# djeedai/bevy_hanabi

Measured on AMD Instinct MI355X. Metric: particle-updates/sec, higher is better.
Workload: dtype f32

## Files before the change

### bevy_hanabi_amd/csrc/hnb_kernels.hip.h

```cpp
#pragma once
#ifndef __HIPCC_RTC__
#include <hip/hip_runtime.h>
#endif
#include "hnb_dev.h"

namespace hnb {

template <class T>
__device__ __forceinline__ T* global_ptr(uint64_t addr) {
    typedef __attribute__((address_space(1))) T global_t;
    return (T*)(global_t*)addr;
}

struct u2_t { uint32_t x, y; };
struct u3_t { uint32_t x, y, z; };
typedef uint32_t u4v __attribute__((ext_vector_type(4)));
#if defined(HNB_NONTEMPORAL) || defined(HNB_NONTEMPORAL_LOADS)
#define HNB_NT_LOAD(p) __builtin_nontemporal_load(p)
#else
#define HNB_NT_LOAD(p) (*(p))
#endif
#if defined(HNB_NONTEMPORAL) || defined(HNB_NONTEMPORAL_STORES)
#define HNB_NT_STORE(v, p) __builtin_nontemporal_store(v, p)
#else
// ... 936 lines not shown
        }
        uint32_t incl = local;
#pragma unroll
        for (uint32_t off = 1; off < 64; off <<= 1) { const uint32_t y = __shfl_up(incl, off, 64); if (lane >= off) incl += y; }
        if (lane == 63) s_scan[wave] = incl;
        __syncthreads();
        uint32_t pos = excl + incl - local;
        for (uint32_t w = 0; w < wave; ++w) pos += s_scan[w];
#pragma unroll
        for (uint32_t r = 0; r < kPer; ++r) {
            if (n_ev[r] >= kEmitHeavy) {
                if ((tid * kPer + r) % n_split == split) {
                    const uint32_t h = atomicAdd(&s_heavy_n, 1u);
                    s_heavy[h][0] = slot[r]; s_heavy[h][1] = pos; s_heavy[h][2] = n_ev[r];
                }
            } else if (split == 0u) {
                const uint32_t end = pos + n_ev[r] < capacity ? pos + n_ev[r] : capacity;
                for (uint32_t e = pos; e < end; ++e) ev->data[e] = slot[r];
            }
            pos += n_ev[r];
        }
        __syncthreads();
        const uint32_t n_heavy = s_heavy_n;
        for (uint32_t h = 0; h < n_heavy; ++h) {
            const uint32_t sl = s_heavy[h][0], first = s_heavy[h][1];
            const uint32_t end = first + s_heavy[h][2] < capacity ? first + s_heavy[h][2] : capacity;
            for (uint32_t e = first + tid; e < end; e += kBlock) ev->data[e] = sl;
        }
        __syncthreads();
    }
}
#endif

#ifndef HNB_STREAM_WAVES
#define HNB_STREAM_WAVES 6
#endif
#ifndef HNB_STREAM_WAVES_FULL
#define HNB_STREAM_WAVES_FULL 5
#endif

template <bool B> struct BoolTag { static constexpr bool value = B; };
struct SlotArgs {
    uint32_t capacity, n_uregs, chunks_per_inst, n_inst;
    soff_t alive_flag_off;
    uint32_t update_len;
    soff_t plane_off[4];
    uint32_t flags;
    soff_t died_bits_off;
    uint32_t write_died;
    uint32_t cull_lifetime;
    soff_t lmin_off;
    uint32_t dt_operand;
    uint32_t age_cohort;
    soff_t horizon_off;
    uint32_t horizon;
    uint32_t frame_phase;
    const Ins* update_code;
    uint32_t* safe_words;
    unsigned long long* safe_host;
    uint32_t safe_parity, publish_tag, safe_stride;
    uint32_t skip_lists;
    const DevMeta* meta_in;
    DevMeta* meta_out;
    uint32_t* fault;
    uint32_t transpose;
    uint32_t stream_hint;
    uint32_t store_hint;
    uint32_t quarters;
    uint32_t age_current;
    uint32_t fuse_steps;
};




__device__ __forceinline__ void store_died_bits(uint32_t* __restrict__ bits, uint32_t step_first, uint32_t nib, uint32_t lane) {
    int v = (int)(nib << (4u * (lane & 7u)));
    v |= __builtin_amdgcn_update_dpp(0, v, 0xB1, 0xf, 0xf, true);
    v |= __builtin_amdgcn_update_dpp(0, v, 0x4E, 0xf, 0xf, true);
    v |= __builtin_amdgcn_update_dpp(0, v, 0x141, 0xf, 0xf, true);
    if ((lane & 7u) == 0u) bits[(step_first >> 5) + (lane >> 3)] = (uint32_t)v;
}

struct StreamLds {
    uint32_t died[kBlock / 64];
    float lmin[kBlock / 64];
    uint32_t alive[kBlock / 64];
    float rem[kBlock / 64];
    uint32_t amin[kBlock / 64], amax[kBlock / 64];
    u4v xp[2][kBlock / 64][kStepRows * 3u / 4u];
};
__device__ __forceinline__ StreamLds& stream_lds() {
    __shared__ StreamLds s;
    return s;
}

template <class PROG, int PROBE, bool COHORT, bool FUSED = false>
__device__ __forceinline__ void update_stream_chunk(const SlotArgs& args, const uint64_t* __restrict__ inst_base, const DevFrameInst* __restrict__ fi,
                                                    const uint32_t* __restrict__ ublocks, const CompactBufs& cb,
                                                    const uint32_t wg, const uint32_t wg_total) {
    StreamLds& lds = stream_lds();
    uint32_t (&s_died)[kBlock / 64] = lds.died;
    float (&s_lmin)[kBlock / 64] = lds.lmin;
    uint32_t (&s_alive)[kBlock / 64] = lds.alive;
    float (&s_rem)[kBlock / 64] = lds.rem;
    uint32_t (&s_amin)[kBlock / 64] = lds.amin;
    uint32_t (&s_amax)[kBlock / 64] = lds.amax;
    u4v (&s_xp)[2][kBlock / 64][kStepRows * 3u / 4u] = lds.xp;
    const uint32_t tid = threadIdx.x, lane = tid & 63u, wave = tid >> 6;
    const bool split = !FUSED && !COHORT && args.quarters == 4u;
    const uint32_t S = FUSED ? args.fuse_steps : 1u;
    const uint32_t chunk = split ? chunk_of_workgroup(cb.xcd_remap, wg >> 2, wg_total >> 2) : chunk_of_workgroup(cb.xcd_remap, wg, wg_total);
    const uint32_t quarter = split ? (wg & 3u) : 0u;
    const uint32_t k = chunk / args.chunks_per_inst, j = chunk - k * args.chunks_per_inst;
    const uint32_t wave0 = j * kChunk + (split ? (quarter * (kBlock / 64u) + wave) * kStepRows : wave * kWaveRows);
    const uint32_t n_steps = split ? 1u : kWaveRows / kStepRows;
    const uint32_t n_words = split ? wg_total >> 2 : wg_total;
    const uint32_t frozen = fi[k].skip;
    const uint64_t slab = inst_base[k];
    const bool store_nt = args.store_hint != 0u;
#ifndef HNB_PUBLISH_FIRST_WG
#define HNB_PUBLISH_FIRST_WG 1
#endif
    if (args.safe_words && (HNB_PUBLISH_FIRST_WG ? wg == 0u : chunk == 0u)) {
        uint32_t* prev = args.safe_words + (size_t)(args.safe_parity ^ 1u) * args.safe_stride;
        uint32_t m = 0x7f800000u;
        for (uint32_t i = tid; i < n_words; i += kBlock) { const uint32_t v = prev[i]; prev[i] = 0x7f800000u; m = v < m ? v : m; }
        m = wave_min_u32(m);
        if (lane == 0) s_alive[wave] = m;
        __syncthreads();
        if (tid == 0u) {
            for (uint32_t w = 1; w < kBlock / 64; ++w) m = s_alive[w] < m ? s_alive[w] : m;
            *reinterpret_cast<volatile unsigned long long*>(args.safe_host) = ((unsigned long long)m << 32) | (unsigned long long)args.publish_tag;
        }
        __syncthreads();
    }
    if (args.skip_lists && j == 0u && quarter == 0u && tid == 0u) {
        DevMeta o = args.meta_in[k];
        if constexpr (FUSED) {
            DevMeta before = o;
            if (!frozen) {
                o.max_update = o.alive_count; o.dead_count = 0u; o.spawned = 0u; o.instance_count = o.alive_count;
                before = o;
                o.ref_write_index ^= S & 1u;
                before.ref_write_index ^= (S - 1u) & 1u;
            }
            DevMeta* row_in = const_cast<DevMeta*>(args.meta_in);
            ((S & 1u) ? args.meta_out : row_in)[k] = o;
            ((S & 1u) ? row_in : args.meta_out)[k] = before;
            cb.deaths[(size_t)(cb.parity ^ 1u) * cb.table_cap + k] = 0u;
        } else {
        if (!frozen) {
            o.ref_write_index ^= 1u;
            o.max_update = o.alive_count; o.dead_count = 0u; o.spawned = 0u; o.instance_count = o.alive_count;
        }
        args.meta_out[k] = o;
        cb.deaths[(size_t)(cb.parity ^ 1u) * cb.table_cap + k] = 0u;
        }
    }
    if (frozen) return;
    char* base = global_ptr<char>(slab);
    VmUniforms U;
    U.u = ublocks + (size_t)k * args.n_uregs * S;
    auto uniforms_of = [&](const uint32_t s) { VmUniforms Us = U; Us.u = U.u + (size_t)s * args.n_uregs; return Us; };
    U.xf = fi[k].xf;
    float rem_min = __builtin_inff();
    char* p_pos = base + args.plane_off[0];
    char* p_vel = base + args.plane_off[1];
    char* p_age = base + args.plane_off[2];
    char* p_life = base + args.plane_off[3];
    uint32_t* flags4 = reinterpret_cast<uint32_t*>(base + args.alive_flag_off);
    const uint32_t fl = args.flags;
    uint32_t died_total = 0;
    uint32_t* cfull = reinterpret_cast<uint32_t*>(base + args.lmin_off) + args.chunks_per_inst;
    const bool chunk_full = cfull[j] == 1u;
    uint32_t* astate = cfull + args.chunks_per_inst;
    uint32_t* aval = astate + args.chunks_per_inst;
    const uint32_t ast_raw = COHORT ? astate[j] : 0u;
    bool check_due = ((args.frame_phase + j) & 15u) == 0u;
    if constexpr (FUSED) {
        for (uint32_t s = 1; s < S; ++s) check_due = check_due || ((args.frame_phase + s + j) & 15u) == 0u;
    }
    const bool mixed = COHORT && ast_raw == 4u && !check_due;
    const uint32_t ast = ast_raw == 4u ? 0u : ast_raw;
    const float A = COHORT ? u2f(aval[j]) : 0.0f;
    uint32_t amin = 0xffffffffu, amax = 0u;
    uint32_t lane_alive = 0;
    const bool cull = args.cull_lifetime != 0u;
    float* lmin = reinterpret_cast<float*>(base + args.lmin_off);
    const float Lm = cull ? lmin[j] : 0.0f;
    const float dt_tick = cull ? uf(U, args.dt_operand) : 0.0f;
    auto age_after = [&](float a) {
        if constexpr (FUSED) {
            for (uint32_t s = 0; s < S; ++s) a = a + uf(uniforms_of(s), args.dt_operand);
            return a;
        } else return a + dt_tick;
    };
    if (args.horizon && j == 0u && quarter == 0u && tid == 0u) {
        double* clk = horizon_view(base, args.horizon_off, args.chunks_per_inst).clock;
        if constexpr (FUSED) {
            double c = *clk;
            for (uint32_t s = 0; s < S; ++s) { const float t = cull ? uf(uniforms_of(s), args.dt_operand) : 0.0f; c = c + (double)(t > 0.0f ? t : 0.0f) * (1.0 + 0x1p-16); }
            *clk = c;
        } else
        *clk = *clk + (double)(dt_tick > 0.0f ? dt_tick : 0.0f) * (1.0 + 0x1p-16);
    }
    float wave_min = __builtin_inff();
    bool loaded_all = true;
    bool flat = false;
    if constexpr (PROG::kFlat && COHORT && PROBE == 0) {
        flat = chunk_full && ast == 1u && cull && Lm > 0.0f && (age_after(A) < Lm) && (fl & 3u) == 3u && !(fl & 128u);
    }
    if (flat) {
        if constexpr (PROG::kFlat && COHORT && PROBE == 0) {
            const float A2 = age_after(A);
            u4v* pw = reinterpret_cast<u4v*>(p_pos + (size_t)j * (kChunk * 12u)) + wave * (kWaveRows * 3u / 4u);
            u4v* vw = reinterpret_cast<u4v*>(p_vel + (size_t)j * (kChunk * 12u)) + wave * (kWaveRows * 3u / 4u);
            const uint32_t rot = lane % 3u;
            if (args.age_current && (fl & 64u)) {
                u4v* aw = reinterpret_cast<u4v*>(p_age + (size_t)j * (kChunk * 4u)) + wave * (kWaveRows / 4u);
                const uint32_t a2 = f2u(A2);
#pragma unroll
                for (uint32_t step = 0; step < kWaveRows / kStepRows; ++step) aw[step * 64u + lane] = u4v{a2, a2, a2, a2};
            }
#pragma unroll 2
            for (uint32_t step = 0; step < kWaveRows / kStepRows; ++step) {
                float P[3][4], V[3][4];
#pragma unroll
                for (uint32_t w = 0; w < 3; ++w) {
                    const u4v a = pw[(step * 3u + w) * 64u + lane], b = vw[(step * 3u + w) * 64u + lane];
                    P[w][0] = u2f(a.x); P[w][1] = u2f(a.y); P[w][2] = u2f(a.z); P[w][3] = u2f(a.w);
                    V[w][0] = u2f(b.x); V[w][1] = u2f(b.y); V[w][2] = u2f(b.z); V[w][3] = u2f(b.w);
                }
                if constexpr (FUSED) {
                    for (uint32_t s = 0; s < S; ++s) PROG::run_flat(args.update_code, P, V, rot, uniforms_of(s));
                } else
                PROG::run_flat(args.update_code, P, V, rot, U);
#pragma unroll
                for (uint32_t w = 0; w < 3; ++w) {
                    if (fl & 16u) pw[(step * 3u + w) * 64u + lane] = u4v{f2u(P[w][0]), f2u(P[w][1]), f2u(P[w][2]), f2u(P[w][3])};
                    if (fl & 32u) vw[(step * 3u + w) * 64u + lane] = u4v{f2u(V[w][0]), f2u(V[w][1]), f2u(V[w][2]), f2u(V[w][3])};
                }
            }
            if (args.write_died && lane < kWaveRows / 32u)
                reinterpret_cast<uint32_t*>(base + args.died_bits_off)[((j * kChunk + wave * kWaveRows) >> 5) + lane] = 0u;
            amin = amax = f2u(A2);
            loaded_all = false;
            if (args.safe_words) rem_min = (f2u(A2) >> 31) ? 0.0f : (Lm - A2) - 1.0e-5f * Lm;
        }
    }
    auto step_body = [&](auto coh_tag, const uint32_t step, const uint32_t f4, const u4v* pre_age = nullptr) {
        constexpr bool COH = decltype(coh_tag)::value;
        const uint32_t s0 = wave0 + step * kStepRows + lane * 4u;
        bool was[4], fresh[4];
#pragma unroll
        for (int p = 0; p < 4; ++p) {
            const uint32_t byte = (f4 >> (8 * p)) & 0xffu;
            fresh[p] = COH && byte == 3u;
            was[p] = byte == 1u || fresh[p];
            lane_alive += was[p] ? 1u : 0u;
        }
        const bool any = was[0] || was[1] || was[2] || was[3];
        if (!__any(any)) {
            if (args.write_died) store_died_bits(reinterpret_cast<uint32_t*>(base + args.died_bits_off), s0 - lane * 4u, 0u, lane);
            return;
        }
        const bool full = was[0] && was[1] && was[2] && was[3];
        uint32_t slot[4];
#pragma unroll
        for (int p = 0; p < 4; ++p) slot[p] = s0 + p;
        bool lanes_on[4] = {any, any, any, any};
        Pinned<4> X;
#pragma unroll
        for (int p = 0; p < 4; ++p) { X.pos[p] = V3{0, 0, 0}; X.vel[p] = V3{0, 0, 0}; X.age[p] = 0.0f; X.lifetime[p] = 0.0f; X.alive[p] = true; }
        bool need_life = true;
        float age_was[4] = {0.0f, 0.0f, 0.0f, 0.0f};
        const uint32_t step_first = s0 - lane * 4u;
        const bool xp = args.transpose != 0u && PROBE == 0 && step_first + kStepRows <= args.capacity && __popcll(__ballot(any)) >= 32;
        if (xp) {
            if (fl & 1u) xpose_load3(X.pos, p_pos, step_first, s_xp[0][wave], lane);
            if (fl & 2u) xpose_load3(X.vel, p_vel, step_first, s_xp[1][wave], lane);
        }
        if (any) {
            if (!xp) {
                if (fl & 1u) pin_load3<4>(X.pos, p_pos, slot, lanes_on, true);
                if (fl & 2u) pin_load3<4>(X.vel, p_vel, slot, lanes_on, true);
            }
            if (fl & 4u) {
                if (!COH || ast != 1u) {
                    if (pre_age) { X.age[0] = u2f(pre_age->x); X.age[1] = u2f(pre_age->y); X.age[2] = u2f(pre_age->z); X.age[3] = u2f(pre_age->w); }
                    else pin_load1<4>(X.age, p_age, slot, lanes_on, true);
                    for (int p = 0; p < 4; ++p) age_was[p] = X.age[p];
                }
                if (COH && ast != 0u) {
#pragma unroll
                    for (int p = 0; p < 4; ++p) X.age[p] = fresh[p] ? X.age[p] : A;
                }
            }
        }
        if (cull && Lm > 0.0f && (COH || !mixed)) {
            bool may_die = false;
#pragma unroll
            for (int p = 0; p < 4; ++p) may_die = may_die || (was[p] && !(age_after(X.age[p]) < Lm));
            need_life = __any(may_die);
        }
        if (any && (fl & 8u)) {
            if (need_life) {
                if (args.stream_hint) {
                    const u4v ql = __builtin_nontemporal_load(reinterpret_cast<const u4v*>(p_life) + (slot[0] >> 2));
                    X.lifetime[0] = u2f(ql.x); X.lifetime[1] = u2f(ql.y); X.lifetime[2] = u2f(ql.z); X.lifetime[3] = u2f(ql.w);
                } else pin_load1<4>(X.lifetime, p_life, slot, lanes_on, true);
            }
            else {
#pragma unroll
                for (int p = 0; p < 4; ++p) X.lifetime[p] = Lm;
            }
        }
        if (!need_life) loaded_all = false;
        if constexpr (FUSED) {
            bool gone[4] = {false, false, false, false};
            for (uint32_t s = 0; s < S; ++s) {
                PROG::template run<4>(args.update_code, args.update_len, X, uniforms_of(s));
#pragma unroll
                for (int p = 0; p < 4; ++p) gone[p] = gone[p] || !X.alive[p];
            }
#pragma unroll
            for (int p = 0; p < 4; ++p) X.alive[p] = !gone[p];
        } else
        if constexpr (!(PROBE & 8)) PROG::template run<4>(args.update_code, args.update_len, X, U);
        if constexpr (!(PROBE & 4)) {
            const bool xp_pos = xp && (fl & 17u) == 17u, xp_vel = xp && (fl & 34u) == 34u;
            if (xp_pos) xpose_store3(X.pos, p_pos, step_first, s_xp[0][wave], lane, was, full, store_nt);
            if (xp_vel) xpose_store3(X.vel, p_vel, step_first, s_xp[1][wave], lane, was, full, store_nt);
            if (any) {
                if ((fl & 16u) && !xp_pos) pin_store3<4>(X.pos, p_pos, slot, was, full);
                if ((fl & 32u) && !xp_vel) pin_store3<4>(X.vel, p_vel, slot, was, full);
                if (fl & 64u) {
                    const bool plane_loaded = !COH || ast != 1u;
                    if (plane_loaded || args.age_current) {
                        if (plane_loaded && (fl & 4u) && !full) {
                            float q[4];
#pragma unroll
                            for (int p = 0; p < 4; ++p) q[p] = was[p] ? X.age[p] : age_was[p];
                            pin_store1<4>(q, p_age, slot, was, true, store_nt);
                        } else pin_store1<4>(X.age, p_age, slot, was, full, store_nt);
                    }
                }
                if (fl & 128u) pin_store1<4>(X.lifetime, p_life, slot, was, full);
            }
        } else {
            float acc = 0.0f;
#pragma unroll
            for (int p = 0; p < 4; ++p) acc += X.pos[p].x + X.pos[p].y + X.pos[p].z + X.vel[p].x + X.vel[p].y + X.vel[p].z + X.age[p] + X.lifetime[p];
            if (acc == 123.456f) X.alive[0] = false;
        }
        if (cull && need_life) {
#pragma unroll
            for (int p = 0; p < 4; ++p)
                if (was[p] && X.alive[p]) wave_min = fminf(wave_min, X.lifetime[p]);
        }
        if (args.safe_words) {
#pragma unroll
            for (int p = 0; p < 4; ++p)
                if (was[p] && X.alive[p]) rem_min = fminf(rem_min, (f2u(X.age[p]) >> 31) ? 0.0f : (X.lifetime[p] - X.age[p]) - 1.0e-5f * X.lifetime[p]);
        }
        if constexpr (COH) {
#pragma unroll
            for (int p = 0; p < 4; ++p) {
                const bool stays = was[p] && X.alive[p];
                const uint32_t b = f2u(X.age[p]);
                amin = (stays && b < amin) ? b : amin;
                amax = (stays && b > amax) ? b : amax;
            }
            if constexpr (!(PROBE & 4)) {
                const bool dies = (was[0] && !X.alive[0]) || (was[1] && !X.alive[1]) || (was[2] && !X.alive[2]) || (was[3] && !X.alive[3]);
                if (ast == 1u && (fl & 64u) && !args.age_current && __any(dies)) {
#pragma unroll
                    for (int p = 0; p < 4; ++p)
                        if (was[p] && !X.alive[p]) reinterpret_cast<float*>(p_age)[slot[p]] = X.age[p];
                }
            }
        }
        uint32_t nf = f4, nib = 0u;
        uint32_t died_here = 0;
#pragma unroll
        for (int p = 0; p < 4; ++p) {
            const bool died = was[p] && !X.alive[p];
            if (died) { nf &= ~(0xffu << (8 * p)); nib |= 1u << p; }
            else if (COH && fresh[p]) nf = (nf & ~(0xffu << (8 * p))) | (1u << (8 * p));
            died_here += (uint32_t)__popcll(__ballot(died));
        }
        if (nf != f4) flags4[s0 >> 2] = nf;
        if (args.write_died) store_died_bits(reinterpret_cast<uint32_t*>(base + args.died_bits_off), step_first, nib, lane);
        died_total += died_here;
    };
    if (!flat) {
        auto f4_of = [&](const uint32_t step) {
            const uint32_t s0 = wave0 + step * kStepRows + lane * 4u;
            return chunk_full ? 0x01010101u : (s0 < args.capacity ? ld_hint(flags4 + (s0 >> 2), args.stream_hint != 0u) : 0u);
        };
        if constexpr (COHORT || PROG::kFlat) {
            uint32_t f4s[kWaveRows / kStepRows];
#pragma unroll
            for (uint32_t step = 0; step < kWaveRows / kStepRows; ++step) f4s[step] = step < n_steps ? f4_of(step) : 0u;
            if constexpr (PROG::kAgeOnly && !COHORT) {
                if ((fl & 4u) && !(fl & 3u)) {
                    u4v ages[kWaveRows / kStepRows];
#pragma unroll
                    for (uint32_t step = 0; step < kWaveRows / kStepRows; ++step) {
                        const uint32_t s0 = wave0 + step * kStepRows + lane * 4u;
                        ages[step] = (step < n_steps && s0 < args.capacity) ? reinterpret_cast<const u4v*>(p_age)[s0 >> 2] : u4v{0u, 0u, 0u, 0u};
                    }
// ... 524 lines not shown
```

### bevy_hanabi_amd/csrc/hnb_vm.h

```cpp
#pragma once
#include "hnb_math.h"
#ifdef __HIPCC_RTC__
#include "hanabi_amd.h"
#else
#include "../../include/hanabi_amd.h"
#endif

namespace hnb {

struct __attribute__((aligned(8))) Ins { uint32_t x, y; };

#ifdef HNB_VM_BOUNDS_CHECK
extern "C" void hnb_vm_oob(uint32_t index, uint32_t size);
template <uint32_t N>
struct checked_file_t {
    uint32_t v[N];
    uint32_t& operator[](uint32_t i) { if (i >= N) hnb_vm_oob(i, N); return v[i < N ? i : 0]; }
    const uint32_t& operator[](uint32_t i) const { if (i >= N) hnb_vm_oob(i, N); return v[i < N ? i : 0]; }
};
typedef checked_file_t<HNB_VM_MAX_REGS> vreg_file_t;
typedef checked_file_t<HNB_VM_MAX_REGS_WIDE> vreg_file_wide_t;
typedef checked_file_t<HNB_VM_MAX_UREGS> UFile;
#else
typedef uint32_t vreg_file_t __attribute__((vector_size(HNB_VM_MAX_REGS * 4)));
// ... 636 lines not shown
template <int P, bool FULL>
HNB_HD void fast_run(const Ins* __restrict__ code, uint32_t n_ins, Pinned<P>& X, const VmUniforms& U) {
    for (uint32_t pc = 0; pc < n_ins; ++pc) {
        const Ins ins = code[pc];
        const uint32_t op = ins.x & 0xffu, d = (ins.x >> 8) & 0xffu, aux = ins.y >> 16;
        const uint32_t a = HNB_OPERAND_DECODE((ins.x >> 16) & 0xffu, ins.y >> 13), b = HNB_OPERAND_DECODE(ins.x >> 24, ins.y >> 14);
        const uint32_t c = HNB_OPERAND_DECODE(ins.y & 0xffu, ins.y >> 15);
        switch (op) {
            case HNB_OP_M_AGE_TICK: {
                const float dt = uf(U, a);
#pragma unroll
                for (int p = 0; p < P; ++p) mac_age_tick(X.age[p], X.lifetime[p], dt, (aux & 1u) != 0u, X.alive[p]);
            } break;
            case HNB_OP_M_EULER: {
                const float dt = uf(U, a);
#pragma unroll
                for (int p = 0; p < P; ++p) mac_euler(X.pos[p], X.vel[p], dt);
            } break;
            case HNB_OP_M_VEL_SCALE: {
                const float s = uf(U, a);
#pragma unroll
                for (int p = 0; p < P; ++p) mac_vel_scale(X.vel[p], s);
            } break;
            case HNB_OP_M_VEL_ADD: {
                const V3 v = uf3(U, a);
#pragma unroll
                for (int p = 0; p < P; ++p) mac_vel_add(X.vel[p], v);
            } break;
            case HNB_OP_M_PIN_SET: {
                if (d == HNB_REG_POSITION || d == HNB_REG_VELOCITY) {
                    const V3 v = uf3(U, a);
#pragma unroll
                    for (int p = 0; p < P; ++p) { if (d == HNB_REG_POSITION) X.pos[p] = v; else X.vel[p] = v; }
                } else {
                    const float s = uf(U, a);
#pragma unroll
                    for (int p = 0; p < P; ++p) { if (d == HNB_REG_AGE) X.age[p] = s; else X.lifetime[p] = s; }
                }
            } break;
            case HNB_OP_M_RADIAL_ACCEL:
                if constexpr (FULL) {
                    const V3 origin = uf3(U, a);
                    const float s = uf(U, b);
#pragma unroll
                    for (int p = 0; p < P; ++p) mac_radial_accel(X.pos[p], X.vel[p], origin, s);
                }
                break;
            case HNB_OP_M_TANGENT_ACCEL:
                if constexpr (FULL) {
                    const V3 origin = uf3(U, a), axis = uf3(U, b);
                    const float s = uf(U, c);
#pragma unroll
                    for (int p = 0; p < P; ++p) mac_tangent_accel(X.pos[p], X.vel[p], origin, axis, s);
                }
                break;
            case HNB_OP_M_CONFORM_SPHERE:
                if constexpr (FULL) {
                    ConformParams q;
                    q.c = uf3(U, a);
                    q.radius = uf(U, a + 3); q.influence_dist = uf(U, a + 4); q.shell_half_thickness = uf(U, a + 5);
                    q.max_attraction_speed = uf(U, a + 6); q.attraction_accel = uf(U, a + 7); q.sticky_factor = uf(U, a + 8);
                    const float dt = uf(U, b);
#pragma unroll
                    for (int p = 0; p < P; ++p) mac_conform_sphere(X.pos[p], X.vel[p], q, dt);
                }
                break;
            case HNB_OP_M_KILL_SPHERE: {
                const V3 center = uf3(U, a);
                const float r2 = uf(U, b);
#pragma unroll
                for (int p = 0; p < P; ++p) mac_kill_sphere(X.pos[p], center, r2, (aux & 1u) != 0u, X.alive[p]);
            } break;
            case HNB_OP_M_KILL_AABB: {
                const V3 center = uf3(U, a), half = uf3(U, b);
#pragma unroll
                for (int p = 0; p < P; ++p) mac_kill_aabb(X.pos[p], center, half, (aux & 1u) != 0u, X.alive[p]);
            } break;
            default: break;
        }
    }
}


template <uint32_t OP, int P>
HNB_HD void apply_static(const Ins ins, Pinned<P>& X, const VmUniforms& U) {
    const uint32_t a = HNB_OPERAND_DECODE((ins.x >> 16) & 0xffu, ins.y >> 13), b = HNB_OPERAND_DECODE(ins.x >> 24, ins.y >> 14);
    const uint32_t c = HNB_OPERAND_DECODE(ins.y & 0xffu, ins.y >> 15), aux = ins.y >> 16;
    if constexpr (OP == HNB_OP_M_AGE_TICK) {
        const float dt = uf(U, a);
        const bool has_lifetime = (aux & 1u) != 0u;
#pragma unroll
        for (int p = 0; p < P; ++p) mac_age_tick(X.age[p], X.lifetime[p], dt, has_lifetime, X.alive[p]);
    } else if constexpr (OP == HNB_OP_M_EULER) {
        const float dt = uf(U, a);
#pragma unroll
        for (int p = 0; p < P; ++p) mac_euler(X.pos[p], X.vel[p], dt);
    } else if constexpr (OP == HNB_OP_M_VEL_SCALE) {
        const float s = uf(U, a);
#pragma unroll
        for (int p = 0; p < P; ++p) mac_vel_scale(X.vel[p], s);
    } else if constexpr (OP == HNB_OP_M_VEL_ADD) {
        const V3 v = uf3(U, a);
#pragma unroll
        for (int p = 0; p < P; ++p) mac_vel_add(X.vel[p], v);
    } else if constexpr (OP == HNB_OP_M_PIN_SET) {
        const uint32_t d = (ins.x >> 8) & 0xffu;
        if (d == HNB_REG_POSITION || d == HNB_REG_VELOCITY) {
            const V3 v = uf3(U, a);
#pragma unroll
            for (int p = 0; p < P; ++p) { if (d == HNB_REG_POSITION) X.pos[p] = v; else X.vel[p] = v; }
        } else {
            const float s = uf(U, a);
#pragma unroll
            for (int p = 0; p < P; ++p) { if (d == HNB_REG_AGE) X.age[p] = s; else X.lifetime[p] = s; }
        }
    } else if constexpr (OP == HNB_OP_M_RADIAL_ACCEL) {
        const V3 origin = uf3(U, a);
        const float s = uf(U, b);
#pragma unroll
        for (int p = 0; p < P; ++p) mac_radial_accel(X.pos[p], X.vel[p], origin, s);
    } else if constexpr (OP == HNB_OP_M_TANGENT_ACCEL) {
        const V3 origin = uf3(U, a), axis = uf3(U, b);
        const float s = uf(U, c);
#pragma unroll
        for (int p = 0; p < P; ++p) mac_tangent_accel(X.pos[p], X.vel[p], origin, axis, s);
    } else if constexpr (OP == HNB_OP_M_CONFORM_SPHERE) {
        ConformParams q;
        q.c = uf3(U, a);
        q.radius = uf(U, a + 3); q.influence_dist = uf(U, a + 4); q.shell_half_thickness = uf(U, a + 5);
        q.max_attraction_speed = uf(U, a + 6); q.attraction_accel = uf(U, a + 7); q.sticky_factor = uf(U, a + 8);
        const float dt = uf(U, b);
#pragma unroll
        for (int p = 0; p < P; ++p) mac_conform_sphere(X.pos[p], X.vel[p], q, dt);
    } else if constexpr (OP == HNB_OP_M_KILL_SPHERE) {
        const V3 center = uf3(U, a);
        const float r2 = uf(U, b);
        const bool inside = (aux & 1u) != 0u;
#pragma unroll
        for (int p = 0; p < P; ++p) mac_kill_sphere(X.pos[p], center, r2, inside, X.alive[p]);
    } else if constexpr (OP == HNB_OP_M_KILL_AABB) {
        const V3 center = uf3(U, a), half = uf3(U, b);
        const bool inside = (aux & 1u) != 0u;
#pragma unroll
        for (int p = 0; p < P; ++p) mac_kill_aabb(X.pos[p], center, half, inside, X.alive[p]);
    } else {
        static_assert(OP == HNB_OP_M_AGE_TICK, "apply_static: opcode is not a streamable macro op");
    }
}

HNB_HD float rot3(const V3 v, uint32_t c) { return c == 0u ? v.x : (c == 1u ? v.y : v.z); }
template <uint32_t OP>
HNB_HD void apply_static_flat(const Ins ins, float (&pos)[3][4], float (&vel)[3][4], uint32_t rot, const VmUniforms& U) {
    const uint32_t a = HNB_OPERAND_DECODE((ins.x >> 16) & 0xffu, ins.y >> 13);
    if constexpr (OP == HNB_OP_M_EULER) {
        const float dt = uf(U, a);
#pragma unroll
        for (int j = 0; j < 3; ++j)
#pragma unroll
            for (int e = 0; e < 4; ++e) pos[j][e] = pos[j][e] + vel[j][e] * dt;
    } else if constexpr (OP == HNB_OP_M_VEL_SCALE) {
        const float s = uf(U, a);
#pragma unroll
        for (int j = 0; j < 3; ++j)
#pragma unroll
            for (int e = 0; e < 4; ++e) vel[j][e] = vel[j][e] * s;
    } else if constexpr (OP == HNB_OP_M_VEL_ADD) {
        const V3 v = uf3(U, a);
        const float vr[3] = {rot3(v, rot % 3u), rot3(v, (rot + 1u) % 3u), rot3(v, (rot + 2u) % 3u)};
#pragma unroll
        for (int j = 0; j < 3; ++j)
#pragma unroll
            for (int e = 0; e < 4; ++e) vel[j][e] = vel[j][e] + vr[(j + e) % 3];
    } else {
        static_assert(OP == HNB_OP_M_AGE_TICK, "apply_static_flat: not a component-wise op");
    }
}

struct ProgInterp {
    static constexpr bool kFlat = false;
    static constexpr bool kAgeOnly = false;
    HNB_HD_MEMBER static void run_flat(const Ins* __restrict__, float (&)[3][4], float (&)[3][4], uint32_t, const VmUniforms&) {}
    static constexpr uint32_t kLen = 0;
    template <int P> HNB_HD_MEMBER static void run(const Ins* __restrict__ code, uint32_t n_ins, Pinned<P>& X, const VmUniforms& U) {
        fast_run<P, true>(code, n_ins, X, U);
    }
};
struct ProgNone {
    static constexpr bool kFlat = false;
    static constexpr bool kAgeOnly = false;
    HNB_HD_MEMBER static void run_flat(const Ins* __restrict__, float (&)[3][4], float (&)[3][4], uint32_t, const VmUniforms&) {}
    static constexpr uint32_t kLen = 0;
    template <int P> HNB_HD_MEMBER static void run(const Ins* __restrict__, uint32_t, Pinned<P>&, const VmUniforms&) {}
    static bool matches(const Ins*, uint32_t n_ins) { return n_ins == 0; }
};
template <uint32_t... OPS>
struct ProgStatic {
    static constexpr uint32_t kLen = sizeof...(OPS);
    static constexpr bool kFlat = ((OPS == HNB_OP_M_AGE_TICK || OPS == HNB_OP_M_EULER || OPS == HNB_OP_M_VEL_SCALE || OPS == HNB_OP_M_VEL_ADD) && ...) &&
                                  ((OPS == HNB_OP_M_AGE_TICK) || ...);
    static constexpr bool kAgeOnly = sizeof...(OPS) > 0 && ((OPS == HNB_OP_M_AGE_TICK) && ...);
    HNB_HD_MEMBER static void run_flat(const Ins* __restrict__ code, float (&pos)[3][4], float (&vel)[3][4], uint32_t rot, const VmUniforms& U) {
        if constexpr (kFlat) {
            uint32_t i = 0;
            ((apply_static_flat<OPS>(code[i++], pos, vel, rot, U)), ...);
        }
    }
    template <int P> HNB_HD_MEMBER static void run(const Ins* __restrict__ code, uint32_t, Pinned<P>& X, const VmUniforms& U) {
        uint32_t i = 0;
        ((apply_static<OPS, P>(code[i++], X, U)), ...);
    }
    static bool matches(const Ins* code, uint32_t n_ins) {
        const uint32_t ops[] = {OPS...};
        if (n_ins != kLen) return false;
        for (uint32_t i = 0; i < kLen; ++i)
            if ((code[i].x & 0xffu) != ops[i]) return false;
        return true;
    }
};

}
```

Before: 126.6 billion.

## Pre-resolve static program uniforms once per chunk and prefetch flat-path loads

Static macro programs now decode their instructions and fetch their uniform operands once per chunk into a small word array. Instructions are read through the constant address space and made wave-uniform, so the per-step loops no longer re-decode operands or re-load uniforms. The flat streaming path gains a variant for the case where both position and velocity are written, which software-pipelines the next step's global loads ahead of the current compute and drops the per-store flag checks. The trade-off is higher register pressure from the pinned resolved words and prefetch buffers, plus more code paths to maintain.

```diff
diff --git a/bevy_hanabi_amd/csrc/hnb_kernels.hip.h b/bevy_hanabi_amd/csrc/hnb_kernels.hip.h
--- a/bevy_hanabi_amd/csrc/hnb_kernels.hip.h
+++ b/bevy_hanabi_amd/csrc/hnb_kernels.hip.h
@@ -1042,6 +1042,12 @@
     if ((lane & 7u) == 0u) bits[(step_first >> 5) + (lane >> 3)] = (uint32_t)v;
 }
 
+#ifndef HNB_FLAT_PREFETCH
+#define HNB_FLAT_PREFETCH 1
+#endif
+#ifndef HNB_FLAT_UNROLL
+#define HNB_FLAT_UNROLL 2
+#endif
 struct StreamLds {
     uint32_t died[kBlock / 64];
     float lmin[kBlock / 64];
@@ -1124,6 +1130,11 @@
     U.u = ublocks + (size_t)k * args.n_uregs * S;
     auto uniforms_of = [&](const uint32_t s) { VmUniforms Us = U; Us.u = U.u + (size_t)s * args.n_uregs; return Us; };
     U.xf = fi[k].xf;
+    const typename PROG::Resolved R = PROG::resolve(args.update_code, U, args.update_len);
+    if constexpr (!FUSED && PROG::kWords != 0u) {
+#pragma unroll
+        for (uint32_t i = 0; i < PROG::kWords; ++i) pin_scalar(R.w[i]);
+    }
     float rem_min = __builtin_inff();
     char* p_pos = base + args.plane_off[0];
     char* p_vel = base + args.plane_off[1];
@@ -1149,7 +1160,7 @@
     const bool cull = args.cull_lifetime != 0u;
     float* lmin = reinterpret_cast<float*>(base + args.lmin_off);
     const float Lm = cull ? lmin[j] : 0.0f;
-    const float dt_tick = cull ? uf(U, args.dt_operand) : 0.0f;
+    const float dt_tick = cull ? ((PROG::kTickFirst && !FUSED) ? PROG::tick(R) : uf(U, args.dt_operand)) : 0.0f;
     auto age_after = [&](float a) {
         if constexpr (FUSED) {
             for (uint32_t s = 0; s < S; ++s) a = a + uf(uniforms_of(s), args.dt_operand);
@@ -1183,25 +1194,55 @@
 #pragma unroll
                 for (uint32_t step = 0; step < kWaveRows / kStepRows; ++step) aw[step * 64u + lane] = u4v{a2, a2, a2, a2};
             }
-#pragma unroll 2
-            for (uint32_t step = 0; step < kWaveRows / kStepRows; ++step) {
-                float P[3][4], V[3][4];
-#pragma unroll
-                for (uint32_t w = 0; w < 3; ++w) {
-                    const u4v a = pw[(step * 3u + w) * 64u + lane], b = vw[(step * 3u + w) * 64u + lane];
-                    P[w][0] = u2f(a.x); P[w][1] = u2f(a.y); P[w][2] = u2f(a.z); P[w][3] = u2f(a.w);
-                    V[w][0] = u2f(b.x); V[w][1] = u2f(b.y); V[w][2] = u2f(b.z); V[w][3] = u2f(b.w);
+            auto flat_steps = [&](auto both_tag) {
+                constexpr bool BOTH = decltype(both_tag)::value;
+                if constexpr (HNB_FLAT_PREFETCH != 0 && BOTH && !FUSED) {
+                    u4v a[3], b[3];
+#pragma unroll
+                    for (uint32_t w = 0; w < 3; ++w) { a[w] = pw[w * 64u + lane]; b[w] = vw[w * 64u + lane]; }
+#pragma unroll
+                    for (uint32_t step = 0; step < kWaveRows / kStepRows; ++step) {
+                        float P[3][4], V[3][4];
+#pragma unroll
+                        for (uint32_t w = 0; w < 3; ++w) {
+                            P[w][0] = u2f(a[w].x); P[w][1] = u2f(a[w].y); P[w][2] = u2f(a[w].z); P[w][3] = u2f(a[w].w);
+                            V[w][0] = u2f(b[w].x); V[w][1] = u2f(b[w].y); V[w][2] = u2f(b[w].z); V[w][3] = u2f(b[w].w);
+                        }
+                        if (step + 1u < kWaveRows / kStepRows) {
+#pragma unroll
+                            for (uint32_t w = 0; w < 3; ++w) { a[w] = pw[((step + 1u) * 3u + w) * 64u + lane]; b[w] = vw[((step + 1u) * 3u + w) * 64u + lane]; }
+                        }
+                        PROG::run_flat(R, P, V, rot);
+#pragma unroll
+                        for (uint32_t w = 0; w < 3; ++w) {
+                            pw[(step * 3u + w) * 64u + lane] = u4v{f2u(P[w][0]), f2u(P[w][1]), f2u(P[w][2]), f2u(P[w][3])};
+                            vw[(step * 3u + w) * 64u + lane] = u4v{f2u(V[w][0]), f2u(V[w][1]), f2u(V[w][2]), f2u(V[w][3])};
+                        }
+                    }
+                    return;
                 }
-                if constexpr (FUSED) {
-                    for (uint32_t s = 0; s < S; ++s) PROG::run_flat(args.update_code, P, V, rot, uniforms_of(s));
-                } else
-                PROG::run_flat(args.update_code, P, V, rot, U);
-#pragma unroll
-                for (uint32_t w = 0; w < 3; ++w) {
-                    if (fl & 16u) pw[(step * 3u + w) * 64u + lane] = u4v{f2u(P[w][0]), f2u(P[w][1]), f2u(P[w][2]), f2u(P[w][3])};
-                    if (fl & 32u) vw[(step * 3u + w) * 64u + lane] = u4v{f2u(V[w][0]), f2u(V[w][1]), f2u(V[w][2]), f2u(V[w][3])};
+#pragma unroll HNB_FLAT_UNROLL
+                for (uint32_t step = 0; step < kWaveRows / kStepRows; ++step) {
+                    float P[3][4], V[3][4];
+#pragma unroll
+                    for (uint32_t w = 0; w < 3; ++w) {
+                        const u4v a = pw[(step * 3u + w) * 64u + lane], b = vw[(step * 3u + w) * 64u + lane];
+                        P[w][0] = u2f(a.x); P[w][1] = u2f(a.y); P[w][2] = u2f(a.z); P[w][3] = u2f(a.w);
+                        V[w][0] = u2f(b.x); V[w][1] = u2f(b.y); V[w][2] = u2f(b.z); V[w][3] = u2f(b.w);
+                    }
+                    if constexpr (FUSED) {
+                        for (uint32_t s = 0; s < S; ++s) PROG::run_flat_each(args.update_code, uniforms_of(s), P, V, rot);
+                    } else
+                    PROG::run_flat(R, P, V, rot);
+#pragma unroll
+                    for (uint32_t w = 0; w < 3; ++w) {
+                        if (BOTH || (fl & 16u)) pw[(step * 3u + w) * 64u + lane] = u4v{f2u(P[w][0]), f2u(P[w][1]), f2u(P[w][2]), f2u(P[w][3])};
+                        if (BOTH || (fl & 32u)) vw[(step * 3u + w) * 64u + lane] = u4v{f2u(V[w][0]), f2u(V[w][1]), f2u(V[w][2]), f2u(V[w][3])};
+                    }
                 }
-            }
+            };
+            if ((fl & 48u) == 48u) flat_steps(BoolTag<true>{});
+            else flat_steps(BoolTag<false>{});
             if (args.write_died && lane < kWaveRows / 32u)
                 reinterpret_cast<uint32_t*>(base + args.died_bits_off)[((j * kChunk + wave * kWaveRows) >> 5) + lane] = 0u;
             amin = amax = f2u(A2);
@@ -1280,14 +1321,14 @@
         if constexpr (FUSED) {
             bool gone[4] = {false, false, false, false};
             for (uint32_t s = 0; s < S; ++s) {
-                PROG::template run<4>(args.update_code, args.update_len, X, uniforms_of(s));
+                PROG::template run_each<4>(args.update_code, args.update_len, uniforms_of(s), X);
 #pragma unroll
                 for (int p = 0; p < 4; ++p) gone[p] = gone[p] || !X.alive[p];
             }
 #pragma unroll
             for (int p = 0; p < 4; ++p) X.alive[p] = !gone[p];
         } else
-        if constexpr (!(PROBE & 8)) PROG::template run<4>(args.update_code, args.update_len, X, U);
+        if constexpr (!(PROBE & 8)) PROG::template run<4>(R, X);
         if constexpr (!(PROBE & 4)) {
             const bool xp_pos = xp && (fl & 17u) == 17u, xp_vel = xp && (fl & 34u) == 34u;
             if (xp_pos) xpose_store3(X.pos, p_pos, step_first, s_xp[0][wave], lane, was, full, store_nt);
diff --git a/bevy_hanabi_amd/csrc/hnb_vm.h b/bevy_hanabi_amd/csrc/hnb_vm.h
--- a/bevy_hanabi_amd/csrc/hnb_vm.h
+++ b/bevy_hanabi_amd/csrc/hnb_vm.h
@@ -742,65 +742,123 @@
 }
 
 
-template <uint32_t OP, int P>
-HNB_HD void apply_static(const Ins ins, Pinned<P>& X, const VmUniforms& U) {
+HNB_HD constexpr uint32_t static_op_words(uint32_t op) {
+    return op == HNB_OP_M_AGE_TICK ? 2u : op == HNB_OP_M_EULER ? 1u : op == HNB_OP_M_VEL_SCALE ? 1u : op == HNB_OP_M_VEL_ADD ? 3u :
+           op == HNB_OP_M_PIN_SET ? 4u : op == HNB_OP_M_RADIAL_ACCEL ? 4u : op == HNB_OP_M_TANGENT_ACCEL ? 7u : op == HNB_OP_M_CONFORM_SPHERE ? 10u :
+           op == HNB_OP_M_KILL_SPHERE ? 5u : op == HNB_OP_M_KILL_AABB ? 7u : 0u;
+}
+HNB_HD uint32_t vm_wave_uniform(uint32_t v) {
+#if defined(__HIP_DEVICE_COMPILE__)
+    return (uint32_t)__builtin_amdgcn_readfirstlane((int)v);
+#else
+    return v;
+#endif
+}
+HNB_HD Ins vm_load_ins(const Ins* p) {
+    Ins r;
+#if defined(__HIP_DEVICE_COMPILE__)
+    typedef const __attribute__((address_space(4))) uint32_t* cptr_t;
+    cptr_t q = (cptr_t)(const uint32_t*)p;
+    r.x = q[0]; r.y = q[1];
+#else
+    r = *p;
+#endif
+    return r;
+}
+template <uint32_t... OPS> constexpr uint32_t static_first_op() { const uint32_t ops[] = {OPS..., 0u}; return ops[0]; }
+HNB_HD V3 w3(const uint32_t* w) { return V3{u2f(w[0]), u2f(w[1]), u2f(w[2])}; }
+HNB_HD void uw3(const VmUniforms& U, uint32_t operand, uint32_t* w) { w[0] = U.u[operand & 0xffu]; w[1] = U.u[(operand + 1) & 0xffu]; w[2] = U.u[(operand + 2) & 0xffu]; }
+
+template <uint32_t OP>
+HNB_HD void resolve_static(const Ins ins, const VmUniforms& U, uint32_t* w) {
     const uint32_t a = HNB_OPERAND_DECODE((ins.x >> 16) & 0xffu, ins.y >> 13), b = HNB_OPERAND_DECODE(ins.x >> 24, ins.y >> 14);
     const uint32_t c = HNB_OPERAND_DECODE(ins.y & 0xffu, ins.y >> 15), aux = ins.y >> 16;
     if constexpr (OP == HNB_OP_M_AGE_TICK) {
-        const float dt = uf(U, a);
-        const bool has_lifetime = (aux & 1u) != 0u;
+        w[0] = U.u[a & 0xffu]; w[1] = aux & 1u;
+    } else if constexpr (OP == HNB_OP_M_EULER || OP == HNB_OP_M_VEL_SCALE) {
+        w[0] = U.u[a & 0xffu];
+    } else if constexpr (OP == HNB_OP_M_VEL_ADD) {
+        uw3(U, a, w);
+    } else if constexpr (OP == HNB_OP_M_PIN_SET) {
+        const uint32_t d = (ins.x >> 8) & 0xffu;
+        w[0] = d;
+        if (d == HNB_REG_POSITION || d == HNB_REG_VELOCITY) uw3(U, a, w + 1);
+        else { w[1] = U.u[a & 0xffu]; w[2] = 0u; w[3] = 0u; }
+    } else if constexpr (OP == HNB_OP_M_RADIAL_ACCEL) {
+        uw3(U, a, w); w[3] = U.u[b & 0xffu];
+    } else if constexpr (OP == HNB_OP_M_TANGENT_ACCEL) {
+        uw3(U, a, w); uw3(U, b, w + 3); w[6] = U.u[c & 0xffu];
+    } else if constexpr (OP == HNB_OP_M_CONFORM_SPHERE) {
+        uw3(U, a, w);
+#pragma unroll
+        for (uint32_t i = 3; i < 9; ++i) w[i] = U.u[(a + i) & 0xffu];
+        w[9] = U.u[b & 0xffu];
+    } else if constexpr (OP == HNB_OP_M_KILL_SPHERE) {
+        uw3(U, a, w); w[3] = U.u[b & 0xffu]; w[4] = aux & 1u;
+    } else if constexpr (OP == HNB_OP_M_KILL_AABB) {
+        uw3(U, a, w); uw3(U, b, w + 3); w[6] = aux & 1u;
+    } else {
+        static_assert(OP == HNB_OP_M_AGE_TICK, "resolve_static: opcode is not a streamable macro op");
+    }
+}
+
+template <uint32_t OP, int P>
+HNB_HD void apply_static(const uint32_t* w, Pinned<P>& X) {
+    if constexpr (OP == HNB_OP_M_AGE_TICK) {
+        const float dt = u2f(w[0]);
+        const bool has_lifetime = w[1] != 0u;
 #pragma unroll
         for (int p = 0; p < P; ++p) mac_age_tick(X.age[p], X.lifetime[p], dt, has_lifetime, X.alive[p]);
     } else if constexpr (OP == HNB_OP_M_EULER) {
-        const float dt = uf(U, a);
+        const float dt = u2f(w[0]);
 #pragma unroll
         for (int p = 0; p < P; ++p) mac_euler(X.pos[p], X.vel[p], dt);
     } else if constexpr (OP == HNB_OP_M_VEL_SCALE) {
-        const float s = uf(U, a);
+        const float s = u2f(w[0]);
 #pragma unroll
         for (int p = 0; p < P; ++p) mac_vel_scale(X.vel[p], s);
     } else if constexpr (OP == HNB_OP_M_VEL_ADD) {
-        const V3 v = uf3(U, a);
+        const V3 v = w3(w);
 #pragma unroll
         for (int p = 0; p < P; ++p) mac_vel_add(X.vel[p], v);
     } else if constexpr (OP == HNB_OP_M_PIN_SET) {
-        const uint32_t d = (ins.x >> 8) & 0xffu;
+        const uint32_t d = w[0];
         if (d == HNB_REG_POSITION || d == HNB_REG_VELOCITY) {
-            const V3 v = uf3(U, a);
+            const V3 v = w3(w + 1);
 #pragma unroll
             for (int p = 0; p < P; ++p) { if (d == HNB_REG_POSITION) X.pos[p] = v; else X.vel[p] = v; }
         } else {
-            const float s = uf(U, a);
+            const float s = u2f(w[1]);
 #pragma unroll
             for (int p = 0; p < P; ++p) { if (d == HNB_REG_AGE) X.age[p] = s; else X.lifetime[p] = s; }
         }
     } else if constexpr (OP == HNB_OP_M_RADIAL_ACCEL) {
-        const V3 origin = uf3(U, a);
-        const float s = uf(U, b);
+        const V3 origin = w3(w);
+        const float s = u2f(w[3]);
 #pragma unroll
         for (int p = 0; p < P; ++p) mac_radial_accel(X.pos[p], X.vel[p], origin, s);
     } else if constexpr (OP == HNB_OP_M_TANGENT_ACCEL) {
-        const V3 origin = uf3(U, a), axis = uf3(U, b);
-        const float s = uf(U, c);
+        const V3 origin = w3(w), axis = w3(w + 3);
+        const float s = u2f(w[6]);
 #pragma unroll
         for (int p = 0; p < P; ++p) mac_tangent_accel(X.pos[p], X.vel[p], origin, axis, s);
     } else if constexpr (OP == HNB_OP_M_CONFORM_SPHERE) {
         ConformParams q;
-        q.c = uf3(U, a);
-        q.radius = uf(U, a + 3); q.influence_dist = uf(U, a + 4); q.shell_half_thickness = uf(U, a + 5);
-        q.max_attraction_speed = uf(U, a + 6); q.attraction_accel = uf(U, a + 7); q.sticky_factor = uf(U, a + 8);
-        const float dt = uf(U, b);
+        q.c = w3(w);
+        q.radius = u2f(w[3]); q.influence_dist = u2f(w[4]); q.shell_half_thickness = u2f(w[5]);
+        q.max_attraction_speed = u2f(w[6]); q.attraction_accel = u2f(w[7]); q.sticky_factor = u2f(w[8]);
+        const float dt = u2f(w[9]);
 #pragma unroll
         for (int p = 0; p < P; ++p) mac_conform_sphere(X.pos[p], X.vel[p], q, dt);
     } else if constexpr (OP == HNB_OP_M_KILL_SPHERE) {
-        const V3 center = uf3(U, a);
-        const float r2 = uf(U, b);
-        const bool inside = (aux & 1u) != 0u;
+        const V3 center = w3(w);
+        const float r2 = u2f(w[3]);
+        const bool inside = w[4] != 0u;
 #pragma unroll
         for (int p = 0; p < P; ++p) mac_kill_sphere(X.pos[p], center, r2, inside, X.alive[p]);
     } else if constexpr (OP == HNB_OP_M_KILL_AABB) {
-        const V3 center = uf3(U, a), half = uf3(U, b);
-        const bool inside = (aux & 1u) != 0u;
+        const V3 center = w3(w), half = w3(w + 3);
+        const bool inside = w[6] != 0u;
 #pragma unroll
         for (int p = 0; p < P; ++p) mac_kill_aabb(X.pos[p], center, half, inside, X.alive[p]);
     } else {
@@ -810,22 +868,21 @@
 
 HNB_HD float rot3(const V3 v, uint32_t c) { return c == 0u ? v.x : (c == 1u ? v.y : v.z); }
 template <uint32_t OP>
-HNB_HD void apply_static_flat(const Ins ins, float (&pos)[3][4], float (&vel)[3][4], uint32_t rot, const VmUniforms& U) {
-    const uint32_t a = HNB_OPERAND_DECODE((ins.x >> 16) & 0xffu, ins.y >> 13);
+HNB_HD void apply_static_flat(const uint32_t* w, float (&pos)[3][4], float (&vel)[3][4], uint32_t rot) {
     if constexpr (OP == HNB_OP_M_EULER) {
-        const float dt = uf(U, a);
+        const float dt = u2f(w[0]);
 #pragma unroll
         for (int j = 0; j < 3; ++j)
 #pragma unroll
             for (int e = 0; e < 4; ++e) pos[j][e] = pos[j][e] + vel[j][e] * dt;
     } else if constexpr (OP == HNB_OP_M_VEL_SCALE) {
-        const float s = uf(U, a);
+        const float s = u2f(w[0]);
 #pragma unroll
         for (int j = 0; j < 3; ++j)
 #pragma unroll
             for (int e = 0; e < 4; ++e) vel[j][e] = vel[j][e] * s;
     } else if constexpr (OP == HNB_OP_M_VEL_ADD) {
-        const V3 v = uf3(U, a);
+        const V3 v = w3(w);
         const float vr[3] = {rot3(v, rot % 3u), rot3(v, (rot + 1u) % 3u), rot3(v, (rot + 2u) % 3u)};
 #pragma unroll
         for (int j = 0; j < 3; ++j)
@@ -836,38 +893,99 @@
     }
 }
 
+template <uint32_t OP, int P>
+HNB_HD void resolve_apply_static(const Ins ins, const VmUniforms& U, Pinned<P>& X) {
+    uint32_t w[static_op_words(OP)];
+    resolve_static<OP>(ins, U, w);
+    apply_static<OP, P>(w, X);
+}
+template <uint32_t OP>
+HNB_HD void resolve_apply_static_flat(const Ins ins, const VmUniforms& U, float (&pos)[3][4], float (&vel)[3][4], uint32_t rot) {
+    uint32_t w[static_op_words(OP)];
+    resolve_static<OP>(ins, U, w);
+    apply_static_flat<OP>(w, pos, vel, rot);
+}
+
 struct ProgInterp {
     static constexpr bool kFlat = false;
     static constexpr bool kAgeOnly = false;
-    HNB_HD_MEMBER static void run_flat(const Ins* __restrict__, float (&)[3][4], float (&)[3][4], uint32_t, const VmUniforms&) {}
+    static constexpr bool kTickFirst = false;
     static constexpr uint32_t kLen = 0;
-    template <int P> HNB_HD_MEMBER static void run(const Ins* __restrict__ code, uint32_t n_ins, Pinned<P>& X, const VmUniforms& U) {
-        fast_run<P, true>(code, n_ins, X, U);
-    }
+    static constexpr uint32_t kWords = 0;
+    struct Resolved { const Ins* code; uint32_t n_ins; VmUniforms U; };
+    HNB_HD_MEMBER static Resolved resolve(const Ins* code, const VmUniforms& U, uint32_t n_ins = 0) { return Resolved{code, n_ins, U}; }
+    HNB_HD_MEMBER static float tick(const Resolved&) { return 0.0f; }
+    HNB_HD_MEMBER static void run_flat(const Resolved&, float (&)[3][4], float (&)[3][4], uint32_t) {}
+    template <int P> HNB_HD_MEMBER static void run(const Resolved& R, Pinned<P>& X) { fast_run<P, true>(R.code, R.n_ins, X, R.U); }
+    HNB_HD_MEMBER static void run_flat_each(const Ins*, const VmUniforms&, float (&)[3][4], float (&)[3][4], uint32_t) {}
+    template <int P> HNB_HD_MEMBER static void run_each(const Ins* code, uint32_t n_ins, const VmUniforms& U, Pinned<P>& X) { fast_run<P, true>(code, n_ins, X, U); }
 };
 struct ProgNone {
     static constexpr bool kFlat = false;
     static constexpr bool kAgeOnly = false;
-    HNB_HD_MEMBER static void run_flat(const Ins* __restrict__, float (&)[3][4], float (&)[3][4], uint32_t, const VmUniforms&) {}
+    static constexpr bool kTickFirst = false;
     static constexpr uint32_t kLen = 0;
-    template <int P> HNB_HD_MEMBER static void run(const Ins* __restrict__, uint32_t, Pinned<P>&, const VmUniforms&) {}
+    static constexpr uint32_t kWords = 0;
+    struct Resolved {};
+    HNB_HD_MEMBER static Resolved resolve(const Ins*, const VmUniforms&, uint32_t = 0) { return Resolved{}; }
+    HNB_HD_MEMBER static float tick(const Resolved&) { return 0.0f; }
+    HNB_HD_MEMBER static void run_flat(const Resolved&, float (&)[3][4], float (&)[3][4], uint32_t) {}
+    template <int P> HNB_HD_MEMBER static void run(const Resolved&, Pinned<P>&) {}
+    HNB_HD_MEMBER static void run_flat_each(const Ins*, const VmUniforms&, float (&)[3][4], float (&)[3][4], uint32_t) {}
+    template <int P> HNB_HD_MEMBER static void run_each(const Ins*, uint32_t, const VmUniforms&, Pinned<P>&) {}
     static bool matches(const Ins*, uint32_t n_ins) { return n_ins == 0; }
 };
 template <uint32_t... OPS>
 struct ProgStatic {
     static constexpr uint32_t kLen = sizeof...(OPS);
+    static constexpr uint32_t kWords = (static_op_words(OPS) + ... + 0u);
     static constexpr bool kFlat = ((OPS == HNB_OP_M_AGE_TICK || OPS == HNB_OP_M_EULER || OPS == HNB_OP_M_VEL_SCALE || OPS == HNB_OP_M_VEL_ADD) && ...) &&
                                   ((OPS == HNB_OP_M_AGE_TICK) || ...);
     static constexpr bool kAgeOnly = sizeof...(OPS) > 0 && ((OPS == HNB_OP_M_AGE_TICK) && ...);
-    HNB_HD_MEMBER static void run_flat(const Ins* __restrict__ code, float (&pos)[3][4], float (&vel)[3][4], uint32_t rot, const VmUniforms& U) {
+    struct Resolved { uint32_t w[kWords ? kWords : 1u]; };
+  private:
+    template <uint32_t OFF> HNB_HD_MEMBER static void resolve_from(const Ins*, const VmUniforms&, uint32_t*) {}
+    template <uint32_t OFF, uint32_t OP, uint32_t... REST> HNB_HD_MEMBER static void resolve_from(const Ins* c, const VmUniforms& U, uint32_t* w) {
+        resolve_static<OP>(c[0], U, w + OFF);
+        resolve_from<OFF + static_op_words(OP), REST...>(c + 1, U, w);
+    }
+    template <int P, uint32_t OFF> HNB_HD_MEMBER static void run_from(const uint32_t*, Pinned<P>&) {}
+    template <int P, uint32_t OFF, uint32_t OP, uint32_t... REST> HNB_HD_MEMBER static void run_from(const uint32_t* w, Pinned<P>& X) {
+        apply_static<OP, P>(w + OFF, X);
+        run_from<P, OFF + static_op_words(OP), REST...>(w, X);
+    }
+    template <uint32_t OFF> HNB_HD_MEMBER static void flat_from(const uint32_t*, float (&)[3][4], float (&)[3][4], uint32_t) {}
+    template <uint32_t OFF, uint32_t OP, uint32_t... REST> HNB_HD_MEMBER static void flat_from(const uint32_t* w, float (&pos)[3][4], float (&vel)[3][4], uint32_t rot) {
+        apply_static_flat<OP>(w + OFF, pos, vel, rot);
+        flat_from<OFF + static_op_words(OP), REST...>(w, pos, vel, rot);
+    }
+  public:
+    static constexpr bool kTickFirst = sizeof...(OPS) > 0 && static_first_op<OPS...>() == HNB_OP_M_AGE_TICK;
+    HNB_HD_MEMBER static Resolved resolve(const Ins* code, const VmUniforms& U, uint32_t = 0) {
+        Ins c[kLen ? kLen : 1u];
+#pragma unroll
+        for (uint32_t i = 0; i < kLen; ++i) c[i] = vm_load_ins(code + i);
+#pragma unroll
+        for (uint32_t i = 0; i < kLen; ++i) { c[i].x = vm_wave_uniform(c[i].x); c[i].y = vm_wave_uniform(c[i].y); }
+        Resolved R;
+        R.w[0] = 0u;
+        resolve_from<0u, OPS...>(c, U, R.w);
+        return R;
+    }
+    HNB_HD_MEMBER static float tick(const Resolved& R) { return u2f(R.w[0]); }
+    HNB_HD_MEMBER static void run_flat(const Resolved& R, float (&pos)[3][4], float (&vel)[3][4], uint32_t rot) {
+        if constexpr (kFlat) flat_from<0u, OPS...>(R.w, pos, vel, rot);
+    }
+    template <int P> HNB_HD_MEMBER static void run(const Resolved& R, Pinned<P>& X) { run_from<P, 0u, OPS...>(R.w, X); }
+    HNB_HD_MEMBER static void run_flat_each(const Ins* code, const VmUniforms& U, float (&pos)[3][4], float (&vel)[3][4], uint32_t rot) {
         if constexpr (kFlat) {
             uint32_t i = 0;
-            ((apply_static_flat<OPS>(code[i++], pos, vel, rot, U)), ...);
+            ((resolve_apply_static_flat<OPS>(vm_load_ins(code + i++), U, pos, vel, rot)), ...);
         }
     }
-    template <int P> HNB_HD_MEMBER static void run(const Ins* __restrict__ code, uint32_t, Pinned<P>& X, const VmUniforms& U) {
+    template <int P> HNB_HD_MEMBER static void run_each(const Ins* code, uint32_t, const VmUniforms& U, Pinned<P>& X) {
         uint32_t i = 0;
-        ((apply_static<OPS, P>(code[i++], X, U)), ...);
+        ((resolve_apply_static<OPS, P>(vm_load_ins(code + i++), U, X)), ...);
     }
     static bool matches(const Ins* code, uint32_t n_ins) {
         const uint32_t ops[] = {OPS...};
```

Result: no change. 126.5 billion (-0.0%).
